# MangoSister/VolumetricTerrain

Measured on AMD Instinct MI355X. Metric: marching-cubes extraction throughput on a 1024^3 perlin3d grid (Mvoxels/s), higher is better.
Workload: dtype f32

## Files before the change

### volumetricterrain_amd/csrc/terrain.hip

```cpp
#include "terrain_edit.h"
#include "terrain_stamp.h"
#include <algorithm>
#include <array>
#include <cmath>
#include <cstring>

namespace vtmc {

__device__ __forceinline__ float clampf(float v, float lo, float hi)
{
    if (v < lo) v = lo;
    else if (v > hi) v = hi;
    return v;
}

__device__ __forceinline__ float lerp_unity(float a, float b, float t)
{
    t = t < 0.0f ? 0.0f : (t > 1.0f ? 1.0f : t);
    return a + (b - a) * t;
}

__device__ __forceinline__ float query_density(const TerrainModifierArgs &m, float px, float py, float pz)
{
    if (m.kind == 0) return m.p[0] - py;
    if (m.kind == 1) {
        const float dx = px - m.p[0], dy = py - m.p[1], dz = pz - m.p[2];
        return m.p[3] - __builtin_sqrtf(dx * dx + dy * dy + dz * dz);
    }
    const float sx = px - m.p[0], sy = py - m.p[1], sz = pz - m.p[2];
    const float proj = sx * m.p[3] + sy * m.p[4] + sz * m.p[5];
    const float sq = sx * sx + sy * sy + sz * sz;
    const float c = m.p[7] - __builtin_sqrtf(sq - proj * proj);
    float r = proj;
    const float b = m.p[6] - proj;
    if (b < r) r = b;
    if (c < r) r = c;
    return r;
}

__global__ __launch_bounds__(256) void terrain_fill_kernel(float *__restrict__ grid, long long n, uint64_t seed)
{
    const long long stride = (long long)gridDim.x * blockDim.x;
    for (long long i = (long long)blockIdx.x * blockDim.x + threadIdx.x; i < n; i += stride)
        grid[i] = terrain_uniform(seed, 0u, (uint64_t)i, 0u) - 2.0f;
}

__device__ __forceinline__ float column_term(const TerrainModifierArgs &m, float px, float pz)
{
    if (m.kind != 3) return 0.0f;
    const float wm1 = (float)(m.dims0 - 1), hm1 = (float)(m.dims1 - 1);
    float u = clampf(px, 0.0f, m.p[0]);
    u = u / m.p[0] * wm1;
    u = clampf(u, 0.0f, wm1);
    float v = clampf(pz, 0.0f, m.p[1]);
    v = v / m.p[1] * hm1;
    v = clampf(v, 0.0f, hm1);
    const int u0 = (int)floorf(u), u1 = (int)ceilf(u), v0 = (int)floorf(v), v1 = (int)ceilf(v);
    const float h00 = m.data[(size_t)u0 * m.dims1 + v0], h10 = m.data[(size_t)u1 * m.dims1 + v0];
    const float h01 = m.data[(size_t)u0 * m.dims1 + v1], h11 = m.data[(size_t)u1 * m.dims1 + v1];
    const float h0 = lerp_unity(h00, h01, v - (float)v0);
    const float h1 = lerp_unity(h10, h11, v - (float)v0);
    return lerp_unity(h0, h1, u - (float)u0);
}

template <bool kJournal>
__global__ __launch_bounds__(256) void terrain_modify_kernel(float *__restrict__ grid, float *__restrict__ image, TerrainShape sh, TerrainModifierArgs m)
{
    const BoxThread t;
    if (!t.inside(m)) return;
    const int x = m.lx + t.ix, z = m.lz + t.iz;
    const float px = (float)x * sh.scale + sh.origin[0];
    const float pz = (float)z * sh.scale + sh.origin[2];
    const float col = column_term(m, px, pz);
    const uint64_t row = box_index(m, t.ix, 0, t.iz);
    for (int iy = t.iy0, iy1 = t.iy1(m); iy < iy1; ++iy) {
        const int y = m.ly + iy;
        const float py = (float)y * sh.scale + sh.origin[1];
        const uint64_t sample = grid_index(sh, x, y, z);
        const float q = m.kind == 3 ? col - py : query_density(m, px, py, pz);
        const float md = clamp_drawn(q, sh.seed, m.event, sample, 0u);
        const float s = grid[sample];
        if (kJournal) image[row + (uint64_t)m.dx * (uint64_t)iy] = s;
        grid[sample] = csg_combine(sh, m.event, sample, m.add_or_erode, md, s);
    }
}

__global__ __launch_bounds__(256) void terrain_swap_kernel(uint32_t *__restrict__ grid, uint32_t *__restrict__ image, TerrainShape sh, TerrainBox b)
{
    const BoxThread t;
    if (!t.inside(b)) return;
    const uint64_t s0 = grid_index(sh, b.lx + t.ix, b.ly + t.iy0, b.lz + t.iz), j0 = box_index(b, t.ix, t.iy0, t.iz);
    const int iy1 = t.iy1(b);
    uint32_t g[kYRun], h[kYRun];
#pragma unroll
    for (int k = 0; k < kYRun; ++k)
        if (t.iy0 + k < iy1) {
            g[k] = grid[s0 + (uint64_t)sh.dim_x * k];
            h[k] = image[j0 + (uint64_t)b.dx * k];
        }
#pragma unroll
    for (int k = 0; k < kYRun; ++k)
        if (t.iy0 + k < iy1) {
            grid[s0 + (uint64_t)sh.dim_x * k] = h[k];
            image[j0 + (uint64_t)b.dx * k] = g[k];
        }
}

__global__ __launch_bounds__(256) void terrain_stage_kernel(const float *__restrict__ grid, float *__restrict__ stage, TerrainShape sh, TerrainBox h)
{
    const BoxThread t;
    if (!t.inside(h)) return;
    const int iy1 = t.iy1(h);
    const uint64_t s0 = grid_index(sh, h.lx + t.ix, h.ly + t.iy0, h.lz + t.iz), j0 = box_index(h, t.ix, t.iy0, t.iz);
    float v[kYRun];
#pragma unroll
    for (int k = 0; k < kYRun; ++k)
        if (t.iy0 + k < iy1) v[k] = grid[s0 + (uint64_t)sh.dim_x * k];
#pragma unroll
    for (int k = 0; k < kYRun; ++k)
        if (t.iy0 + k < iy1) stage[j0 + (uint64_t)h.dx * k] = v[k];
}

hipError_t launch_terrain_fill(float *grid, long long n, uint64_t seed, int n_cus, hipStream_t stream)
{
    long long wgs = (n + 255) / 256;
    if (wgs > (long long)n_cus * 16) wgs = (long long)n_cus * 16;
    if (wgs < 1) wgs = 1;
    return launch(terrain_fill_kernel, dim3((unsigned)wgs), dim3(256), 0, stream, grid, n, seed);
}

hipError_t launch_terrain_modify(float *grid, const TerrainShape &sh, const TerrainModifierArgs &m, hipStream_t stream)
{
    return box_empty(box_of(m)) ? hipSuccess : launch_box(terrain_modify_kernel<false>, box_of(m), stream, grid, (float *)nullptr, sh, m);
}

hipError_t launch_terrain_copy_box(const float *grid, float *dst, const TerrainShape &sh, const TerrainBox &b, hipStream_t stream)
{
    return launch_box(terrain_stage_kernel, b, stream, grid, dst, sh, b);
}

static int saturating_int(float f)
{
    return f <= -2147483648.0f ? INT32_MIN : (f >= 2147483648.0f ? INT32_MAX : (int)f);
}

static std::array<int, 3> block_counts(const TerrainShape &sh) { return {(sh.dim_x - 2) / 8, (sh.dim_y - 2) / 8, (sh.dim_z - 2) / 8}; }
template <class F>
static void for_each_block(const std::array<int, 3> &nb, F f)
{
    for (int bz = 0; bz < nb[2]; ++bz)
        for (int by = 0; by < nb[1]; ++by)
            for (int bx = 0; bx < nb[0]; ++bx) f(bx, by, bz);
}

TerrainModifierArgs sample_range(const TerrainShape &sh, const vtmc_modifier &md, int low[3], int up[3])
{
    TerrainModifierArgs a{};
    a.kind = md.kind;
    a.add_or_erode = md.add_or_erode ? 1 : 0;
    memcpy(a.p, md.p, sizeof a.p);
    const int top[3] = {sh.dim_x - 1, sh.dim_y - 1, sh.dim_z - 1};
    int ext[3];
    for (int k = 0; k < 3; ++k) {
        low[k] = std::max(saturating_int(std::floor((md.lower[k] - sh.origin[k]) / sh.scale)), 0);
        up[k] = std::min(saturating_int(std::ceil((md.upper[k] - sh.origin[k]) / sh.scale)), top[k]);
        const long long e = (long long)up[k] - (long long)low[k] + 1;
        ext[k] = e <= 0 || low[k] > top[k] ? 0 : (int)std::min<long long>(e, (long long)top[k] - low[k] + 1);
    }
    a.lx = low[0], a.ly = low[1], a.lz = low[2];
    a.dx = ext[0], a.dy = ext[1], a.dz = ext[2];
    return a;
}

TerrainBox bounds_box(const TerrainShape &sh, const float lower[3], const float upper[3])
{
    vtmc_modifier md{};
    for (int k = 0; k < 3; ++k) md.lower[k] = lower[k], md.upper[k] = upper[k];
    int low[3], up[3];
    return box_of(sample_range(sh, md, low, up));
}

static size_t mark_dirty_blocks(const int low[3], const int up[3], const std::array<int, 3> &nb, std::vector<uint8_t> &mark)
{
    int b0[3], b1[3];
    for (int k = 0; k < 3; ++k) {
        const long long lo = (long long)low[k] - 8, hi = up[k];
        const long long f = lo <= 0 ? 0 : (lo + 7) / 8;
        const long long l = std::min<long long>(hi < 0 ? -1 : hi / 8, nb[k] - 1);
        if (f > l) return 0;
        b0[k] = (int)f;
        b1[k] = (int)l;
    }
    size_t n_new = 0;
    for (int bz = b0[2]; bz <= b1[2]; ++bz)
        for (int by = b0[1]; by <= b1[1]; ++by) {
            uint8_t *row = &mark[(size_t)nb[0] * ((size_t)by + (size_t)nb[1] * bz)];
            for (int bx = b0[0]; bx <= b1[0]; ++bx) {
                n_new += !row[bx];
                row[bx] = 1;
            }
        }
    return n_new;
}

int stage_for_queue(vtmc_ctx *ctx, VtmcDevBuf &buf, const void *host, size_t bytes)
{
    VTMC_HIP(ctx, hipStreamSynchronize(ctx->stream));
    if (int rc = ensure(ctx, buf, bytes)) return rc;
    VTMC_HIP(ctx, hipMemcpy(buf.p, host, bytes, hipMemcpyHostToDevice));
    return VTMC_OK;
}

static int check_reference(vtmc_ctx *ctx, const vtmc_modifier &md, int32_t i)
{
    if (md.kind == VTMC_MOD_HEIGHTMAP && (!md.data || md.data_dims[0] < 1 || md.data_dims[1] < 1))
        return fail(ctx, VTMC_ERR_INVALID_ARG, "modifier %d: heightmap data / dims missing", i);
    return VTMC_OK;
}

static int apply_reference(vtmc_ctx *ctx, const vtmc_modifier &md, const TerrainModifierArgs &args, float *grid, float *image)
{
    TerrainModifierArgs a = args;
    if (md.kind == VTMC_MOD_HEIGHTMAP) {
        if (int rc = stage_for_queue(ctx, ctx->heightmap, md.data, sizeof(float) * (size_t)md.data_dims[0] * (size_t)md.data_dims[1])) return rc;
        a.data = (const float *)ctx->heightmap.p;
        a.dims0 = md.data_dims[0];
        a.dims1 = md.data_dims[1];
    }
    VTMC_HIP(ctx, launch_box(image ? terrain_modify_kernel<true> : terrain_modify_kernel<false>, box_of(a), ctx->stream, grid, image, ctx->tshape, a));
    return VTMC_OK;
}

static const ModifierKind kModifierKinds[] = {
    {VTMC_MOD_PLANE, check_reference, apply_reference},
    {VTMC_MOD_SPHERE, check_reference, apply_reference},
    {VTMC_MOD_CYLINDER, check_reference, apply_reference},
    {VTMC_MOD_HEIGHTMAP, check_reference, apply_reference},
    {VTMC_MOD_SMOOTH, check_brush, apply_smooth},
    {VTMC_MOD_FLATTEN, check_brush, apply_flatten},
    {VTMC_MOD_NOISE, check_noise, apply_noise},
    {VTMC_MOD_STAMP, check_stamp, apply_stamp},
    {VTMC_MOD_PATH, check_path, apply_path},
    {VTMC_MOD_DETACH, check_detach, apply_detach},
};

const ModifierKind *find_modifier_kind(int32_t kind)
{
    for (const ModifierKind &k : kModifierKinds)
        if (k.kind == kind) return &k;
    return nullptr;
}

static int check_modifier(vtmc_ctx *ctx, const vtmc_modifier &md, int32_t i)
{
    const ModifierKind *k = find_modifier_kind(md.kind);
    return k ? k->check(ctx, md, i) : fail(ctx, VTMC_ERR_INVALID_ARG, "modifier %d: unknown kind %d", i, md.kind);
}

static int extract_dirty(vtmc_ctx *ctx, const std::vector<uint8_t> &mark, size_t n_marked, int32_t *n_dirty_blocks, int32_t *tri_count)
{
    const TerrainShape &sh = ctx->tshape;
    const auto nb = block_counts(sh);
    ctx->dirty.clear();
    ctx->dirty_is_all = n_marked == mark.size();
    if (!ctx->dirty_is_all) {
        ctx->dirty.reserve(n_marked * 3);
        size_t id = 0;
        for_each_block(nb, [&](int bx, int by, int bz) {
            if (mark[id++]) ctx->dirty.insert(ctx->dirty.end(), {bx, by, bz});
        });
    }
    if (n_dirty_blocks) *n_dirty_blocks = (int32_t)n_marked;
    BlockSpace sp = dense_space((const float *)ctx->terrain.p, sh.dim_x - 2, sh.dim_y - 2, sh.dim_z - 2, 1, sh.dim_x, (int64_t)sh.dim_x * sh.dim_y, 1, 0);
    int n_volumes = 1;
    if (!ctx->dirty_is_all) {
        if (int rc = upload_block_list(ctx, ctx->dirty.data(), (int)n_marked, sp)) return rc;
        n_volumes = 0;
    }
    return extract_core(ctx, sp, n_volumes, ResultSource::TerrainDirty, tri_count);
}

void history_clear(vtmc_ctx *ctx)
{
    ctx->hist.clear();
    ctx->hist_done = 0;
}

int terrain_extract_all(vtmc_ctx *ctx, int32_t *n_dirty_blocks, int32_t *tri_count)
{
    const auto nb = block_counts(ctx->tshape);
    const std::vector<uint8_t> mark((size_t)nb[0] * nb[1] * nb[2], 1);
    return extract_dirty(ctx, mark, mark.size(), n_dirty_blocks, tri_count);
}

static size_t image_bytes(const TerrainBox &b) { return box_empty(b) ? 0 : ((size_t)4 * b.dx * b.dy * b.dz + 255) / 256 * 256; }

static VtmcHistoryStep plan_step(vtmc_ctx *ctx, const vtmc_modifier *mods, int32_t n_mods)
{
    VtmcHistoryStep st;
    st.boxes.resize((size_t)n_mods);
    for (int32_t i = 0; i < n_mods; ++i) {
        VtmcHistoryBox &hb = st.boxes[i];
        const TerrainModifierArgs a = sample_range(ctx->tshape, mods[i], hb.low, hb.up);
        hb.box = box_of(a);
        hb.off = st.bytes;
        st.bytes += image_bytes(hb.box);
    }
    const size_t cap = ctx->journal.bytes;
    if (st.bytes == 0 || st.bytes > cap) {
        if (st.bytes) history_clear(ctx);
        st.boxes.clear();
        return st;
    }
    ctx->hist.resize(ctx->hist_done);
    const size_t head = ctx->hist.empty() ? 0 : ctx->hist.back().off + ctx->hist.back().bytes;
    st.off = head + st.bytes <= cap ? head : 0;
    if (st.off == 0)
        while (!ctx->hist.empty() && ctx->hist.front().off >= head) ctx->hist.pop_front();
    while (!ctx->hist.empty() && ctx->hist.front().off < st.off + st.bytes && st.off < ctx->hist.front().off + ctx->hist.front().bytes)
        ctx->hist.pop_front();
    ctx->hist_done = ctx->hist.size();
    for (VtmcHistoryBox &hb : st.boxes) hb.off += st.off;
    return st;
}

static int32_t history_step(vtmc_ctx *ctx, bool undo, int32_t *n_dirty_blocks, int32_t *tri_count)
{
    if (!ctx) return VTMC_ERR_INVALID_ARG;
    if (!ctx->has_terrain) return fail(ctx, VTMC_ERR_NO_RESULT, "terrain_%s before terrain_init", undo ? "undo" : "redo");
    if (undo ? ctx->hist_done == 0 : ctx->hist_done == ctx->hist.size())
        return fail(ctx, VTMC_ERR_NO_RESULT, "nothing to %s", undo ? "undo" : "redo");
    VTMC_HIP(ctx, hipSetDevice(ctx->device));
    const size_t k = undo ? ctx->hist_done - 1 : ctx->hist_done;
    const VtmcHistoryStep &st = ctx->hist[k];
    const auto nb = block_counts(ctx->tshape);
    std::vector<uint8_t> mark((size_t)nb[0] * nb[1] * nb[2], 0);
    size_t n_marked = 0;
    const size_t n = st.boxes.size();
    for (size_t i = 0; i < n; ++i) {
        const VtmcHistoryBox &hb = st.boxes[undo ? n - 1 - i : i];
        if (!box_empty(hb.box))
            if (hipError_t e = launch_box(terrain_swap_kernel, hb.box, ctx->stream, (uint32_t *)ctx->terrain.p,
                                          (uint32_t *)((char *)ctx->journal.p + hb.off), ctx->tshape, hb.box)) {
                history_clear(ctx);
                VTMC_HIP(ctx, e);
            }
        if (n_marked < mark.size()) n_marked += mark_dirty_blocks(hb.low, hb.up, nb, mark);
    }
    ctx->hist_done = undo ? k : k + 1;
    return extract_dirty(ctx, mark, n_marked, n_dirty_blocks, tri_count);
}

}

using namespace vtmc;

extern "C" {

int32_t vtmc_terrain_init(vtmc_ctx *ctx, int32_t width, int32_t elevation, int32_t height, float voxel_scale,
                          const float terrain_origin[3], uint64_t seed)
{
    if (!ctx) return VTMC_ERR_INVALID_ARG;
    if (!terrain_origin) return fail(ctx, VTMC_ERR_INVALID_ARG, "terrain_origin is null");
    if (int rc = check_dims(ctx, width, elevation, height)) return rc;
    if (width + 1 > 1025 || elevation + 1 > 1025 || height + 1 > 1025)
        return fail(ctx, VTMC_ERR_DIMS, "too high resolution (exceeds 1025)");
    if (!(voxel_scale > 0.0f)) return fail(ctx, VTMC_ERR_INVALID_ARG, "voxel_scale must be positive");
    VTMC_HIP(ctx, hipSetDevice(ctx->device));
    ctx->has_terrain = false;
    ctx->result.valid = false;
    history_clear(ctx);
    material_drop(ctx);
    nav_drop(ctx);
    water_drop(ctx);
    TerrainShape sh{};
    sh.dim_x = width + 2;
    sh.dim_y = elevation + 2;
    sh.dim_z = height + 2;
    sh.scale = voxel_scale;
    memcpy(sh.origin, terrain_origin, sizeof sh.origin);
    sh.seed = seed;
    const long long n = (long long)sh.dim_x * sh.dim_y * sh.dim_z;
    if (int rc = ensure(ctx, ctx->terrain, sizeof(float) * (size_t)n)) return rc;
    VTMC_HIP(ctx, launch_terrain_fill((float *)ctx->terrain.p, n, seed, ctx->n_cus, ctx->stream));
    VTMC_HIP(ctx, hipStreamSynchronize(ctx->stream));
    ctx->tshape = sh;
    ctx->terrain_events = 0;
    ctx->dirty.clear();
    ctx->dirty_is_all = false;
    ctx->has_terrain = true;
    return VTMC_OK;
}

int32_t vtmc_terrain_update(vtmc_ctx *ctx, const vtmc_modifier *mods, int32_t n_mods, int32_t *n_dirty_blocks, int32_t *tri_count)
{
    if (!ctx) return VTMC_ERR_INVALID_ARG;
    if (!ctx->has_terrain) return fail(ctx, VTMC_ERR_NO_RESULT, "terrain_update before terrain_init");
    if (n_mods < 0 || (n_mods > 0 && !mods)) return fail(ctx, VTMC_ERR_INVALID_ARG, "mods is null or n_mods < 0");
    VTMC_HIP(ctx, hipSetDevice(ctx->device));
    const TerrainShape &sh = ctx->tshape;
    const auto nb = block_counts(sh);
    std::vector<uint8_t> mark((size_t)nb[0] * nb[1] * nb[2], 0);
    size_t n_marked = 0;
    VtmcHistoryStep step;
    if (ctx->journal.p) {
        for (int32_t i = 0; i < n_mods; ++i)
            if (int rc = check_modifier(ctx, mods[i], i)) return rc;
        step = plan_step(ctx, mods, n_mods);
    }
    const bool journaled = !step.boxes.empty();
    struct ClearOnFailure {
        vtmc_ctx *ctx;
        bool armed;
        ~ClearOnFailure()
        {
            if (armed) history_clear(ctx);
        }
    } guard{ctx, journaled};
    for (int32_t i = 0; i < n_mods; ++i) {
        const vtmc_modifier &md = mods[i];
        if (int rc = check_modifier(ctx, md, i)) return rc;
        int low[3], up[3];
        TerrainModifierArgs a = sample_range(sh, md, low, up);
        a.event = ++ctx->terrain_events;
        if (!box_empty(box_of(a))) {
            float *image = journaled ? (float *)((char *)ctx->journal.p + step.boxes[i].off) : nullptr;
            if (int rc = find_modifier_kind(md.kind)->apply(ctx, md, a, (float *)ctx->terrain.p, image)) return rc;
        }
        if (n_marked < mark.size()) n_marked += mark_dirty_blocks(low, up, nb, mark);
    }
    if (journaled) {
        ctx->hist.push_back(std::move(step));
        ctx->hist_done = ctx->hist.size();
    }
    const int rc = extract_dirty(ctx, mark, n_marked, n_dirty_blocks, tri_count);
    guard.armed = rc != VTMC_OK && journaled;
    return rc;
}

int32_t vtmc_terrain_set_history(vtmc_ctx *ctx, int64_t max_bytes)
{
    if (!ctx) return VTMC_ERR_INVALID_ARG;
    if (max_bytes < 0) return fail(ctx, VTMC_ERR_INVALID_ARG, "max_bytes < 0");
    VTMC_HIP(ctx, hipSetDevice(ctx->device));
    history_clear(ctx);
    if (ctx->journal.bytes != (size_t)max_bytes) {
        VTMC_HIP(ctx, hipStreamSynchronize(ctx->stream));
        ctx->journal.release();
        if (max_bytes > 0) {
            VTMC_HIP(ctx, hipMalloc(&ctx->journal.p, (size_t)max_bytes));
            ctx->journal.bytes = (size_t)max_bytes;
        }
    }
    return VTMC_OK;
}

int32_t vtmc_terrain_undo(vtmc_ctx *ctx, int32_t *n_dirty_blocks, int32_t *tri_count) { return history_step(ctx, true, n_dirty_blocks, tri_count); }

int32_t vtmc_terrain_redo(vtmc_ctx *ctx, int32_t *n_dirty_blocks, int32_t *tri_count) { return history_step(ctx, false, n_dirty_blocks, tri_count); }

int32_t vtmc_terrain_history(const vtmc_ctx *ctx, int32_t *n_undo, int32_t *n_redo, int64_t *bytes_used)
{
    if (!ctx) return VTMC_ERR_INVALID_ARG;
    if (n_undo) *n_undo = (int32_t)ctx->hist_done;
    if (n_redo) *n_redo = (int32_t)(ctx->hist.size() - ctx->hist_done);
    if (bytes_used) {
        int64_t b = 0;
        for (const VtmcHistoryStep &st : ctx->hist) b += (int64_t)st.bytes;
        *bytes_used = b;
    }
    return VTMC_OK;
}

int32_t vtmc_terrain_dirty_blocks(vtmc_ctx *ctx, int32_t *dst, int32_t capacity_blocks, int32_t *n_blocks)
{
    if (!ctx) return VTMC_ERR_INVALID_ARG;
    if (!ctx->has_terrain) return fail(ctx, VTMC_ERR_NO_RESULT, "terrain_dirty_blocks before terrain_init");
    const auto nb = block_counts(ctx->tshape);
    const size_t n = ctx->dirty_is_all ? (size_t)nb[0] * nb[1] * nb[2] : ctx->dirty.size() / 3;
    if (n_blocks) *n_blocks = (int32_t)n;
    if (!dst) return VTMC_OK;
    if ((size_t)std::max(capacity_blocks, 0) < n) return fail(ctx, VTMC_ERR_CAPACITY, "capacity %d < %zu dirty blocks", capacity_blocks, n);
    if (ctx->dirty_is_all)
        for_each_block(nb, [&](int bx, int by, int bz) {
            *dst++ = bx;
            *dst++ = by;
            *dst++ = bz;
        });
    else if (n)
        memcpy(dst, ctx->dirty.data(), n * 3 * sizeof(int32_t));
    return VTMC_OK;
}

int32_t vtmc_terrain_read_samples(vtmc_ctx *ctx, float *dst, int64_t stride_x, int64_t stride_y, int64_t stride_z)
{
    if (!ctx) return VTMC_ERR_INVALID_ARG;
    if (!ctx->has_terrain) return fail(ctx, VTMC_ERR_NO_RESULT, "terrain_read_samples before terrain_init");
    if (!dst) return fail(ctx, VTMC_ERR_INVALID_ARG, "dst is null");
    if (stride_x <= 0 || stride_y <= 0 || stride_z <= 0) return fail(ctx, VTMC_ERR_INVALID_ARG, "strides must be positive");
    VTMC_HIP(ctx, hipSetDevice(ctx->device));
    const TerrainShape &sh = ctx->tshape;
    const size_t n = (size_t)sh.dim_x * sh.dim_y * sh.dim_z;
    VTMC_HIP(ctx, hipStreamSynchronize(ctx->stream));
    if (stride_x == 1 && stride_y == sh.dim_x && stride_z == (int64_t)sh.dim_x * sh.dim_y) {
        VTMC_HIP(ctx, hipMemcpy(dst, ctx->terrain.p, n * sizeof(float), hipMemcpyDeviceToHost));
        return VTMC_OK;
    }
    std::vector<float> tmp(n);
    VTMC_HIP(ctx, hipMemcpy(tmp.data(), ctx->terrain.p, n * sizeof(float), hipMemcpyDeviceToHost));
    size_t i = 0;
    for (int z = 0; z < sh.dim_z; ++z)
        for (int y = 0; y < sh.dim_y; ++y)
            for (int x = 0; x < sh.dim_x; ++x) dst[x * stride_x + y * stride_y + z * stride_z] = tmp[i++];
    return VTMC_OK;
}

int32_t vtmc_terrain_device_grid(vtmc_ctx *ctx, const float **d_samples, int64_t strides[3], int32_t dims[3])
{
    if (!ctx) return VTMC_ERR_INVALID_ARG;
    if (!ctx->has_terrain) return fail(ctx, VTMC_ERR_NO_RESULT, "terrain_device_grid before terrain_init");
    const TerrainShape &sh = ctx->tshape;
    if (d_samples) *d_samples = (const float *)ctx->terrain.p;
    if (strides) {
        strides[0] = 1;
        strides[1] = sh.dim_x;
        strides[2] = (int64_t)sh.dim_x * sh.dim_y;
    }
    if (dims) {
        dims[0] = sh.dim_x;
        dims[1] = sh.dim_y;
        dims[2] = sh.dim_z;
    }
    return VTMC_OK;
}

}
```

### volumetricterrain_amd/csrc/terrain_box.h

```cpp
#ifndef VTMC_TERRAIN_BOX_H
#define VTMC_TERRAIN_BOX_H
#include "vtmc_ctx.h"
#include "terrain_hash.h"

namespace vtmc {

__device__ __forceinline__ float clamp_drawn(float v, uint64_t seed, uint32_t event, uint64_t sample, uint32_t k)
{
    if (v < -1.0f) {
        const float lo = terrain_uniform(seed, event, sample, k) - 2.0f;
        if (v < lo) v = lo;
    } else if (v > 1.0f) {
        const float hi = terrain_uniform(seed, event, sample, k + 1u) + 1.0f;
        if (v > hi) v = hi;
    }
    return v;
}

__device__ __forceinline__ float csg_combine(const TerrainShape &sh, uint32_t event, uint64_t sample, int add_or_erode, float md, float s)
{
    if (add_or_erode) return s > md ? s : md;
    const float minus_md = -md;
    return clamp_drawn(s < minus_md ? s : minus_md, sh.seed, event, sample, 2u);
}

constexpr int kYRun = 16;

struct BoxThread {
    int ix, iz, iy0;
    __device__ __forceinline__ BoxThread() : ix(blockIdx.x * 64 + threadIdx.x), iz(blockIdx.y * 4 + threadIdx.y), iy0(blockIdx.z * kYRun) {}
    template <class Box>
    __device__ __forceinline__ bool inside(const Box &b) const { return ix < b.dx && iz < b.dz; }
    template <class Box>
    __device__ __forceinline__ int iy1(const Box &b) const { return iy0 + kYRun < b.dy ? iy0 + kYRun : b.dy; }
};
__device__ __forceinline__ uint64_t grid_index(const TerrainShape &sh, int x, int y, int z)
{
    return (uint64_t)x + (uint64_t)sh.dim_x * ((uint64_t)y + (uint64_t)sh.dim_y * (uint64_t)z);
}
template <class Box>
__device__ __forceinline__ uint64_t box_index(const Box &b, int ix, int iy, int iz)
{
    return (uint64_t)ix + (uint64_t)b.dx * ((uint64_t)iy + (uint64_t)b.dy * (uint64_t)iz);
}

static bool box_empty(const TerrainBox &b) { return b.dx <= 0 || b.dy <= 0 || b.dz <= 0; }

static dim3 box_grid(const TerrainBox &b) { return dim3((unsigned)((b.dx + 63) / 64), (unsigned)((b.dz + 3) / 4), (unsigned)((b.dy + kYRun - 1) / kYRun)); }
static bool box_launchable(const TerrainBox &b) { return (b.dz + 3) / 4 <= 65535 && (b.dy + kYRun - 1) / kYRun <= 65535; }

template <class... Params, class... Args>
static hipError_t launch_box(void (*kernel)(Params...), const TerrainBox &b, hipStream_t stream, Args... args)
{
    return box_launchable(b) ? launch(kernel, box_grid(b), dim3(64, 4, 1), 0, stream, args...) : hipErrorInvalidValue;
}

}
#endif
```

### volumetricterrain_amd/csrc/terrain_edit.h

```cpp
#ifndef VTMC_TERRAIN_EDIT_H
#define VTMC_TERRAIN_EDIT_H
#include "terrain_box.h"

namespace vtmc {

struct ModifierKind {
    int32_t kind;
    int (*check)(vtmc_ctx *ctx, const vtmc_modifier &md, int32_t i);
    int (*apply)(vtmc_ctx *ctx, const vtmc_modifier &md, const TerrainModifierArgs &a, float *grid, float *image);
};
const ModifierKind *find_modifier_kind(int32_t kind);

int check_brush(vtmc_ctx *ctx, const vtmc_modifier &md, int32_t i);
int check_noise(vtmc_ctx *ctx, const vtmc_modifier &md, int32_t i);
int check_stamp(vtmc_ctx *ctx, const vtmc_modifier &md, int32_t i);
int check_path(vtmc_ctx *ctx, const vtmc_modifier &md, int32_t i);
int check_detach(vtmc_ctx *ctx, const vtmc_modifier &md, int32_t i);
int apply_smooth(vtmc_ctx *ctx, const vtmc_modifier &md, const TerrainModifierArgs &a, float *grid, float *image);
int apply_flatten(vtmc_ctx *ctx, const vtmc_modifier &md, const TerrainModifierArgs &a, float *grid, float *image);
int apply_noise(vtmc_ctx *ctx, const vtmc_modifier &md, const TerrainModifierArgs &a, float *grid, float *image);
int apply_stamp(vtmc_ctx *ctx, const vtmc_modifier &md, const TerrainModifierArgs &a, float *grid, float *image);
int apply_path(vtmc_ctx *ctx, const vtmc_modifier &md, const TerrainModifierArgs &a, float *grid, float *image);
int apply_detach(vtmc_ctx *ctx, const vtmc_modifier &md, const TerrainModifierArgs &a, float *grid, float *image);

static TerrainBox box_of(const TerrainModifierArgs &m) { return TerrainBox{m.lx, m.ly, m.lz, m.dx, m.dy, m.dz}; }
TerrainModifierArgs sample_range(const TerrainShape &sh, const vtmc_modifier &md, int low[3], int up[3]);
TerrainBox bounds_box(const TerrainShape &sh, const float lower[3], const float upper[3]);
int stage_for_queue(vtmc_ctx *ctx, VtmcDevBuf &buf, const void *host, size_t bytes);

}
#endif
```

### volumetricterrain_amd/csrc/vtmc_ctx.h

```cpp
#ifndef VTMC_CTX_H
#define VTMC_CTX_H
#include "../../include/vtmc.h"
#include "vtmc_internal.h"
struct vtmc_nav_span;
#include "../../include/vtmc_water.h"

#include <deque>
#include <map>
#include <string>
#include <utility>
#include <vector>

namespace vtmc {
struct TerrainBox {
    int lx, ly, lz;
    int dx, dy, dz;
};
template <typename T, hipError_t (*Free)(void *)>
struct OwnedBuf {
    T *p = nullptr;
    size_t bytes = 0;
    OwnedBuf() = default;
    OwnedBuf(OwnedBuf &&o) noexcept { swap(o); }
    OwnedBuf &operator=(OwnedBuf o) noexcept { return swap(o); }
    ~OwnedBuf() { release(); }
    OwnedBuf &swap(OwnedBuf &o) noexcept
    {
        std::swap(p, o.p);
        std::swap(bytes, o.bytes);
        return *this;
    }
    void release()
    {
        if (p) quiet(Free(p));
        p = nullptr;
        bytes = 0;
    }
};
template <int N>
struct StageClock {
    hipEvent_t ev[N] = {};
    bool armed = false;
    StageClock() = default;
    StageClock(const StageClock &) = delete;
    StageClock &operator=(const StageClock &) = delete;
    ~StageClock()
    {
        for (hipEvent_t e : ev)
            if (e) quiet(hipEventDestroy(e));
    }
    hipError_t begin()
    {
        armed = false;
        for (hipEvent_t &e : ev)
            if (!e)
                if (hipError_t rc = hipEventCreate(&e)) return rc;
        return hipSuccess;
    }
    hipError_t mark(int i, hipStream_t stream) { return hipEventRecord(ev[i], stream); }
    void arm() { armed = true; }
    hipEvent_t event(int i) const { return ev[i]; }
    int sync_last(vtmc_ctx *ctx) const;
    int elapsed(vtmc_ctx *ctx, int i, int j, float *ms) const;
};
}
typedef vtmc::OwnedBuf<void, hipFree> VtmcDevBuf;
template <typename T>
using VtmcPinnedBuf = vtmc::OwnedBuf<T, hipHostFree>;

struct VtmcHistoryBox {
    vtmc::TerrainBox box;
    int low[3], up[3];
    size_t off = 0;
};
struct VtmcHistoryStep {
    std::vector<VtmcHistoryBox> boxes;
    size_t off = 0, bytes = 0;
};

struct VtmcStamp {
    VtmcDevBuf samples;
    int nx = 0, ny = 0, nz = 0;
};

enum class ResultSource { Caller, TerrainDirty, TerrainLod };

struct VtmcResult {
    bool valid = false;
    uint64_t epoch = 0;
    ResultSource source = ResultSource::Caller;
    vtmc::BlockSpace space{};
    int blocks = 0;
    uint32_t active = 0;
    int volumes = 0;
    int64_t tris = 0, verts = 0;
    bool indexed = false;
    int64_t vertices() const { return indexed ? verts : 3 * tris; }
};

struct VertexAttr {
    VtmcDevBuf values;
    int64_t n = 0;
    uint64_t epoch = 0;
};

struct VtmcScatter {
    VtmcDevBuf instances, block_offsets, masks, tiles;
    int64_t n = 0;
    int blocks = 0;
    uint64_t epoch = 0;
};

struct VtmcNav {
    VtmcDevBuf spans, offsets, scan, scratch, ctl;
    VtmcDevBuf spans_next, offsets_next;
    bool valid = false;
    int32_t n = 0;
    int32_t lo[3] = {0, 0, 0}, d[3] = {0, 0, 0};
    int rounds = 0;
};

struct VtmcNavField {
    VtmcDevBuf cells, work, ctl;
    bool valid = false;
    int32_t n = 0, reached = 0, rounds = 0;
};

struct VtmcNavErode {
    VtmcDevBuf state, links, dist, remap, origin, ctl;
    bool dist_valid = false, origin_valid = false;
    int32_t dist_n = 0, origin_n = 0;
    int32_t rounds = 0;
};

struct VtmcNavCrowd {
    VtmcDevBuf agents, pending, occupancy, claims, links, ctl;
    bool valid = false;
    int32_t n_agents = 0, n_spans = 0;
    int32_t occupying = 0, arrived = 0, ticks = 0, moved_last = 0;
};

struct VtmcWater {
    VtmcDevBuf water, body, labels, records, seeds, source_body, ctl, probe;
    bool valid = false;
    int32_t lo[3] = {0, 0, 0}, d[3] = {0, 0, 0}, vd[3] = {0, 0, 0};
    int64_t wet = 0;
    std::vector<vtmc_water_body> bodies;
};

struct VtmcLodSkirt {
    VtmcDevBuf tris, node_offsets, masks, tiles, node_masks, sink;
    std::vector<uint8_t> face_masks;
    int64_t n = 0;
    int32_t nodes = 0, flagged = 0;
    uint64_t epoch = 0;
    bool staged = false;
};

struct VtmcPending {
    bool active = false;
    bool launched = false;
    vtmc::BlockSpace sp{};
    int n_volumes = 0;
    bool indexed = false;
    ResultSource source = ResultSource::Caller;
    hipStream_t stream = nullptr;
    size_t tcap = 0, vcap = 0;
    bool scan_event = false;
    bool counts_early = false;
};

struct vtmc_ctx {
    int device = 0;
    int n_cus = 256;
    hipStream_t stream = nullptr;
    bool stream_own_queue = false;
    hipStream_t queue_stream = nullptr;
    vtmc::DeviceTables tables{nullptr, nullptr};
    VtmcDevBuf d_vert, d_trinum;
    VtmcDevBuf counts, offsets, active, partials, totals, volcounts, cases, tris, input, list, perm, origins, yrows;
    VtmcDevBuf vcounts, voffsets, vtotals, verts, indices;
    int output_mode = VTMC_OUTPUT_SOUP;
    uint32_t *h_totals_dev = nullptr;
    VtmcPinnedBuf<uint32_t> h_totals;
    hipEvent_t ev[5] = {nullptr, nullptr, nullptr, nullptr, nullptr};
    VtmcDevBuf signs;
    struct {
        bool valid = false;
        const float *d_out = nullptr;
        int dx = 0, dy = 0, dz = 0, n_volumes = 0;
        long long sv = 0;
    } sign_of;
    VtmcPinnedBuf<float> h_stage;
    int h_stage_small_calls = 0;
    VtmcPinnedBuf<int32_t> h_origins;
    hipEvent_t ev_origins = nullptr;
    bool origins_upload_pending = false;
    float stage_ms[4] = {0, 0, 0, 0};
    bool place_pending = false;
    float place_ms[16] = {0, 0, 0, 0, 0, 0, 0, 0, 0, 0, 0, 0, 0, 0, 0, 0};
    int place_n = 0, place_kept = 0;
    vtmc::StageClock<2> fill_clock;
    VtmcPending pending;
    VtmcResult result;
    vtmc::Tuning tune;
    VtmcDevBuf terrain, heightmap;
    vtmc::TerrainShape tshape{};
    bool has_terrain = false;
    uint32_t terrain_events = 0;
    std::vector<int32_t> dirty;
    bool dirty_is_all = false;
    VtmcDevBuf journal;
    std::deque<VtmcHistoryStep> hist;
    size_t hist_done = 0;
    VtmcDevBuf brush;
    std::map<int32_t, VtmcStamp> stamps;
    int32_t next_stamp_id = 1;
    VtmcDevBuf path;
    VtmcDevBuf frag_labels, frag_ctl, frag_records;
    VtmcDevBuf material, mat_image, mat_strokes;
    int mat_c = 0;
    VertexAttr mat_weights;
    VertexAttr ao;
    VtmcDevBuf ao_stats;
    int32_t ao_direct_max = -1;
    VtmcScatter scatter;
    vtmc::StageClock<6> scatter_clock;
    VtmcNav nav;
    vtmc::StageClock<9> nav_clock;
    VtmcNavField navfield;
    vtmc::StageClock<4> navfield_clock;
    VtmcNavErode naverode;
    vtmc::StageClock<5> naverode_clock;
    VtmcDevBuf navsight_links;
    vtmc::StageClock<3> navsight_clock;
    VtmcNavCrowd navcrowd;
    vtmc::StageClock<2> navcrowd_clock;
    VtmcWater water;
    vtmc::StageClock<4> water_clock;
    std::vector<vtmc_lod_node> lod_nodes;
    VtmcDevBuf lod_nodes_dev, lod_tiles;
    vtmc::StageClock<2> lod_clock;
    VtmcLodSkirt lodskirt;
    vtmc::StageClock<6> lodskirt_clock;
    VtmcDevBuf rays;
    VtmcPinnedBuf<unsigned char> h_rays;
    uint64_t perm_seed = 0;
    bool perm_valid = false;
    VtmcDevBuf tio_bricks, tio_stage;
    VtmcPinnedBuf<unsigned char> h_tio;
    VtmcDevBuf chunk_image;
    bool comm_borrowed = false;
    void *comm = nullptr;
    int comm_rank = 0, comm_world = 1;
    VtmcDevBuf comm_send;
    hipStream_t comm_stream = nullptr;
    hipEvent_t ev_gather = nullptr;
    hipEvent_t ev_last_gather = nullptr;
    bool gather_recorded = false;
    hipEvent_t ev_comm_chain = nullptr;
    hipStream_t comm_chain_stream = nullptr;
    bool comm_chain_recorded = false;
    vtmc_ctx *comm_owner = nullptr;
    std::vector<vtmc_ctx *> comm_borrowers;
    std::string err;
};

namespace vtmc {
int fail(vtmc_ctx *ctx, int code, const char *fmt, ...) __attribute__((format(printf, 3, 4)));
int ensure(vtmc_ctx *ctx, VtmcDevBuf &b, size_t bytes);
inline void release(VtmcDevBuf &b) { b.release(); }
template <typename T>
hipError_t pin(VtmcPinnedBuf<T> &b, size_t bytes)
{
    b.release();
    const hipError_t e = hipHostMalloc((void **)&b.p, bytes, hipHostMallocDefault);
    if (e == hipSuccess) b.bytes = bytes;
    else b.p = nullptr;
    return e;
}
hipError_t take_stream(int device, bool own_queue, int n_cus, hipStream_t *out);
void comm_release(vtmc_ctx *ctx);
int check_dims(vtmc_ctx *ctx, int nx, int ny, int nz);
BlockSpace dense_space(const float *d_base, int nx, int ny, int nz, int64_t sx, int64_t sy, int64_t sz, int n_volumes, int64_t sv);
float *pinned_stage(vtmc_ctx *ctx, size_t bytes);
void material_drop(vtmc_ctx *ctx);
inline void nav_drop(vtmc_ctx *ctx) { ctx->nav.valid = false, ctx->navfield.valid = false, ctx->naverode.dist_valid = false, ctx->naverode.origin_valid = false, ctx->navcrowd.valid = false; }
inline void water_drop(vtmc_ctx *ctx) { ctx->water.valid = false; }
int upload_block_list(vtmc_ctx *ctx, const int32_t *xyz, int n, BlockSpace &sp);
int extract_core(vtmc_ctx *ctx, const BlockSpace &sp, int n_volumes, ResultSource source, int32_t *tri_count);
int attr_gate(vtmc_ctx *ctx, const char *who);
int attr_read(vtmc_ctx *ctx, const VertexAttr &a, const char *stale, size_t bytes_per_vertex, uint8_t *dst, int64_t capacity_vertices);
int attr_device_results(vtmc_ctx *ctx, const VertexAttr &a, const char *stale, const uint8_t **d_values, int64_t *n_vertices);
void history_clear(vtmc_ctx *ctx);
int terrain_extract_all(vtmc_ctx *ctx, int32_t *n_dirty_blocks, int32_t *tri_count);

struct ScanLayout;
hipError_t nav_launch_offsets(const ScanLayout &scan, int32_t *offsets, hipStream_t stream);
int nav_label_regions(vtmc_ctx *ctx, const char *who, vtmc_nav_span *spans, int32_t *parent, int32_t n, bool timed, int *rounds);
struct NavBox;
NavBox nav_held_box(const VtmcNav &nav);

struct TraceRows {
    const int32_t *starts;
    int32_t *paths, *lengths;
    size_t path_bytes, length_bytes, host_off;
};
int trace_rows_stage(vtmc_ctx *ctx, const int32_t *starts, int32_t n_starts, int32_t max_len, TraceRows *rows);
int trace_rows_fetch(vtmc_ctx *ctx, const TraceRows &rows, int32_t *paths, int32_t *lengths);

template <class... Params, class... Args>
hipError_t launch(void (*kernel)(Params...), dim3 grid, dim3 block, size_t lds_bytes, hipStream_t stream, Args... args)
{
    launch_begin();
    hipLaunchKernelGGL(kernel, grid, block, lds_bytes, stream, args...);
    return launch_end();
}
inline dim3 lanes256(int64_t n) { return dim3((unsigned)((n + 255) / 256)); }
}

#define VTMC_HIP(ctx, expr)                                                                                \
    do {                                                                                                   \
        hipError_t e_ = (expr);                                                                            \
        if (e_ != hipSuccess)                                                                              \
            return vtmc::fail(ctx, VTMC_ERR_DEVICE, "%s failed: %s (%s:%d)", #expr, hipGetErrorString(e_), \
                              __FILE__, __LINE__);                                                         \
    } while (0)

template <int N>
int vtmc::StageClock<N>::sync_last(vtmc_ctx *ctx) const
{
    VTMC_HIP(ctx, hipSetDevice(ctx->device));
    VTMC_HIP(ctx, hipEventSynchronize(ev[N - 1]));
    return VTMC_OK;
}
template <int N>
int vtmc::StageClock<N>::elapsed(vtmc_ctx *ctx, int i, int j, float *ms) const
{
    VTMC_HIP(ctx, hipEventElapsedTime(ms, ev[i], ev[j]));
    return VTMC_OK;
}

#endif
```

Baseline: 663,400.

## Batch non-overlapping plane/sphere/cylinder terrain modifiers into one kernel launch

Plane, sphere and cylinder modifiers are now queued instead of launched one at a time. They are grouped into dependency levels by box overlap, and up to sixteen modifiers per level go out in a single batched kernel that maps blocks to modifiers through prefix offsets. The modify kernel also loads its y-run of grid samples up front before computing. This targets launch overhead in terrain editing. The metric is marching-cubes extraction throughput, which this path likely does not touch, and the batching adds host-side reordering and per-block modifier lookup.

Measured after the change: 647,300. 2.4% lower.

```diff
diff --git a/volumetricterrain_amd/csrc/terrain.hip b/volumetricterrain_amd/csrc/terrain.hip
--- a/volumetricterrain_amd/csrc/terrain.hip
+++ b/volumetricterrain_amd/csrc/terrain.hip
@@ -64,25 +64,52 @@
 }
 
 template <bool kJournal>
-__global__ __launch_bounds__(256) void terrain_modify_kernel(float *__restrict__ grid, float *__restrict__ image, TerrainShape sh, TerrainModifierArgs m)
-{
-    const BoxThread t;
+__device__ __forceinline__ void modify_run(float *__restrict__ grid, float *__restrict__ image, const TerrainShape &sh, const TerrainModifierArgs &m, const BoxThread &t)
+{
     if (!t.inside(m)) return;
     const int x = m.lx + t.ix, z = m.lz + t.iz;
     const float px = (float)x * sh.scale + sh.origin[0];
     const float pz = (float)z * sh.scale + sh.origin[2];
     const float col = column_term(m, px, pz);
-    const uint64_t row = box_index(m, t.ix, 0, t.iz);
-    for (int iy = t.iy0, iy1 = t.iy1(m); iy < iy1; ++iy) {
-        const int y = m.ly + iy;
-        const float py = (float)y * sh.scale + sh.origin[1];
-        const uint64_t sample = grid_index(sh, x, y, z);
-        const float q = m.kind == 3 ? col - py : query_density(m, px, py, pz);
-        const float md = clamp_drawn(q, sh.seed, m.event, sample, 0u);
-        const float s = grid[sample];
-        if (kJournal) image[row + (uint64_t)m.dx * (uint64_t)iy] = s;
-        grid[sample] = csg_combine(sh, m.event, sample, m.add_or_erode, md, s);
-    }
+    const int n = t.iy1(m) - t.iy0;
+    const uint64_t s0 = grid_index(sh, x, m.ly + t.iy0, z);
+    const uint64_t j0 = box_index(m, t.ix, t.iy0, t.iz);
+    float s[kYRun];
+    load_run(s, grid + s0, (uint64_t)sh.dim_x, n);
+#pragma unroll
+    for (int k = 0; k < kYRun; ++k)
+        if (k < n) {
+            const int y = m.ly + t.iy0 + k;
+            const float py = (float)y * sh.scale + sh.origin[1];
+            const uint64_t sample = s0 + (uint64_t)sh.dim_x * k;
+            const float q = m.kind == 3 ? col - py : query_density(m, px, py, pz);
+            const float md = clamp_drawn(q, sh.seed, m.event, sample, 0u);
+            if (kJournal) image[j0 + (uint64_t)m.dx * k] = s[k];
+            grid[sample] = csg_combine(sh, m.event, sample, m.add_or_erode, md, s[k]);
+        }
+}
+
+template <bool kJournal>
+__global__ __launch_bounds__(256) void terrain_modify_kernel(float *__restrict__ grid, float *__restrict__ image, TerrainShape sh, TerrainModifierArgs m)
+{
+    modify_run<kJournal>(grid, image, sh, m, BoxThread());
+}
+
+constexpr int kModifyBatch = 16;
+struct ModifyBatch {
+    TerrainModifierArgs m[kModifyBatch];
+    float *image[kModifyBatch];
+    unsigned first[kModifyBatch];
+};
+template <bool kJournal>
+__global__ __launch_bounds__(256) void terrain_modify_batch_kernel(float *__restrict__ grid, TerrainShape sh, ModifyBatch b)
+{
+    int j = 0;
+#pragma unroll
+    for (int k = 1; k < kModifyBatch; ++k) j += blockIdx.x >= b.first[k];
+    const TerrainModifierArgs &m = b.m[j];
+    const unsigned w = blockIdx.x - b.first[j], gx = (unsigned)(m.dx + 63) / 64, gz = (unsigned)(m.dz + 3) / 4;
+    modify_run<kJournal>(grid, kJournal ? b.image[j] : nullptr, sh, m, BoxThread(w % gx, w / gx % gz, w / gx / gz));
 }
 
 __global__ __launch_bounds__(256) void terrain_swap_kernel(uint32_t *__restrict__ grid, uint32_t *__restrict__ image, TerrainShape sh, TerrainBox b)
@@ -218,24 +245,77 @@
     return VTMC_OK;
 }
 
-static int apply_reference(vtmc_ctx *ctx, const vtmc_modifier &md, const TerrainModifierArgs &args, float *grid, float *image)
+static hipError_t launch_modify(vtmc_ctx *ctx, const TerrainModifierArgs &a, float *image)
+{
+    return launch_box(image ? terrain_modify_kernel<true> : terrain_modify_kernel<false>, box_of(a), ctx->stream, (float *)ctx->terrain.p, image, ctx->tshape, a);
+}
+
+static int apply_heightmap(vtmc_ctx *ctx, const vtmc_modifier &md, const TerrainModifierArgs &args, float *, float *image)
 {
     TerrainModifierArgs a = args;
-    if (md.kind == VTMC_MOD_HEIGHTMAP) {
-        if (int rc = stage_for_queue(ctx, ctx->heightmap, md.data, sizeof(float) * (size_t)md.data_dims[0] * (size_t)md.data_dims[1])) return rc;
-        a.data = (const float *)ctx->heightmap.p;
-        a.dims0 = md.data_dims[0];
-        a.dims1 = md.data_dims[1];
-    }
-    VTMC_HIP(ctx, launch_box(image ? terrain_modify_kernel<true> : terrain_modify_kernel<false>, box_of(a), ctx->stream, grid, image, ctx->tshape, a));
+    if (int rc = stage_for_queue(ctx, ctx->heightmap, md.data, sizeof(float) * (size_t)md.data_dims[0] * (size_t)md.data_dims[1])) return rc;
+    a.data = (const float *)ctx->heightmap.p;
+    a.dims0 = md.data_dims[0];
+    a.dims1 = md.data_dims[1];
+    VTMC_HIP(ctx, launch_modify(ctx, a, image));
+    return VTMC_OK;
+}
+
+static int apply_reference(vtmc_ctx *ctx, const vtmc_modifier &, const TerrainModifierArgs &a, float *, float *image)
+{
+    ctx->stretch.push_back({a, image});
+    return VTMC_OK;
+}
+
+static bool boxes_overlap(const TerrainModifierArgs &a, const TerrainModifierArgs &b)
+{
+    return a.lx < b.lx + b.dx && b.lx < a.lx + a.dx && a.ly < b.ly + b.dy && b.ly < a.ly + a.dy && a.lz < b.lz + b.dz && b.lz < a.lz + a.dz;
+}
+
+static int flush_stretch(vtmc_ctx *ctx)
+{
+    std::vector<VtmcQueuedModifier> q;
+    q.swap(ctx->stretch);
+    const size_t n = q.size();
+    std::vector<int> level(n, 0);
+    std::vector<size_t> order(n);
+    for (size_t i = 0; i < n; ++i) {
+        order[i] = i;
+        for (size_t j = 0; j < i; ++j)
+            if (level[j] >= level[i] && boxes_overlap(q[j].a, q[i].a)) level[i] = level[j] + 1;
+    }
+    std::stable_sort(order.begin(), order.end(), [&](size_t x, size_t y) { return level[x] < level[y]; });
+    for (size_t at = 0; at < n;) {
+        ModifyBatch b{};
+        uint64_t wgs = 0;
+        size_t k = 0;
+        for (; k < kModifyBatch && at + k < n && level[order[at + k]] == level[order[at]]; ++k) {
+            const VtmcQueuedModifier &qm = q[order[at + k]];
+            const dim3 g = box_grid(box_of(qm.a));
+            const uint64_t own = (uint64_t)g.x * g.y * g.z;
+            if (k > 0 && wgs + own > 0x7fffffffu) break;
+            b.m[k] = qm.a;
+            b.image[k] = qm.image;
+            b.first[k] = (unsigned)wgs;
+            wgs += own;
+        }
+        if (k == 1) {
+            VTMC_HIP(ctx, launch_modify(ctx, b.m[0], b.image[0]));
+        } else {
+            for (size_t r = k; r < kModifyBatch; ++r) b.first[r] = UINT32_MAX;
+            VTMC_HIP(ctx, launch(b.image[0] ? terrain_modify_batch_kernel<true> : terrain_modify_batch_kernel<false>, dim3((unsigned)wgs), dim3(64, 4, 1), 0,
+                                 ctx->stream, (float *)ctx->terrain.p, ctx->tshape, b));
+        }
+        at += k;
+    }
     return VTMC_OK;
 }
 
 static const ModifierKind kModifierKinds[] = {
-    {VTMC_MOD_PLANE, check_reference, apply_reference},
-    {VTMC_MOD_SPHERE, check_reference, apply_reference},
-    {VTMC_MOD_CYLINDER, check_reference, apply_reference},
-    {VTMC_MOD_HEIGHTMAP, check_reference, apply_reference},
+    {VTMC_MOD_PLANE, check_reference, apply_reference, true},
+    {VTMC_MOD_SPHERE, check_reference, apply_reference, true},
+    {VTMC_MOD_CYLINDER, check_reference, apply_reference, true},
+    {VTMC_MOD_HEIGHTMAP, check_reference, apply_heightmap},
     {VTMC_MOD_SMOOTH, check_brush, apply_smooth},
     {VTMC_MOD_FLATTEN, check_brush, apply_flatten},
     {VTMC_MOD_NOISE, check_noise, apply_noise},
@@ -417,18 +497,27 @@
             if (armed) history_clear(ctx);
         }
     } guard{ctx, journaled};
-    for (int32_t i = 0; i < n_mods; ++i) {
-        const vtmc_modifier &md = mods[i];
-        if (int rc = check_modifier(ctx, md, i)) return rc;
-        int low[3], up[3];
-        TerrainModifierArgs a = sample_range(sh, md, low, up);
-        a.event = ++ctx->terrain_events;
-        if (!box_empty(box_of(a))) {
-            float *image = journaled ? (float *)((char *)ctx->journal.p + step.boxes[i].off) : nullptr;
-            if (int rc = find_modifier_kind(md.kind)->apply(ctx, md, a, (float *)ctx->terrain.p, image)) return rc;
-        }
-        if (n_marked < mark.size()) n_marked += mark_dirty_blocks(low, up, nb, mark);
-    }
+    const auto walk = [&]() -> int {
+        for (int32_t i = 0; i < n_mods; ++i) {
+            const vtmc_modifier &md = mods[i];
+            if (int rc = check_modifier(ctx, md, i)) return rc;
+            const ModifierKind *kind = find_modifier_kind(md.kind);
+            if (!kind->enqueues)
+                if (int rc = flush_stretch(ctx)) return rc;
+            int low[3], up[3];
+            TerrainModifierArgs a = sample_range(sh, md, low, up);
+            a.event = ++ctx->terrain_events;
+            if (!box_empty(box_of(a))) {
+                float *image = journaled ? (float *)((char *)ctx->journal.p + step.boxes[i].off) : nullptr;
+                if (int rc = kind->apply(ctx, md, a, (float *)ctx->terrain.p, image)) return rc;
+            }
+            if (n_marked < mark.size()) n_marked += mark_dirty_blocks(low, up, nb, mark);
+        }
+        return VTMC_OK;
+    };
+    const int walked = walk(), flushed = flush_stretch(ctx);
+    if (walked) return walked;
+    if (flushed) return flushed;
     if (journaled) {
         ctx->hist.push_back(std::move(step));
         ctx->hist_done = ctx->hist.size();
diff --git a/volumetricterrain_amd/csrc/terrain_box.h b/volumetricterrain_amd/csrc/terrain_box.h
--- a/volumetricterrain_amd/csrc/terrain_box.h
+++ b/volumetricterrain_amd/csrc/terrain_box.h
@@ -28,7 +28,8 @@
 
 struct BoxThread {
     int ix, iz, iy0;
-    __device__ __forceinline__ BoxThread() : ix(blockIdx.x * 64 + threadIdx.x), iz(blockIdx.y * 4 + threadIdx.y), iy0(blockIdx.z * kYRun) {}
+    __device__ __forceinline__ BoxThread() : BoxThread(blockIdx.x, blockIdx.y, blockIdx.z) {}
+    __device__ __forceinline__ BoxThread(unsigned bx, unsigned bz, unsigned by) : ix(bx * 64 + threadIdx.x), iz(bz * 4 + threadIdx.y), iy0(by * kYRun) {}
     template <class Box>
     __device__ __forceinline__ bool inside(const Box &b) const { return ix < b.dx && iz < b.dz; }
     template <class Box>
@@ -44,6 +45,14 @@
     return (uint64_t)ix + (uint64_t)b.dx * ((uint64_t)iy + (uint64_t)b.dy * (uint64_t)iz);
 }
 
+template <class T>
+__device__ __forceinline__ void load_run(T (&v)[kYRun], const T *p, uint64_t stride, int n)
+{
+#pragma unroll
+    for (int k = 0; k < kYRun; ++k)
+        if (k < n) v[k] = p[stride * k];
+}
+
 static bool box_empty(const TerrainBox &b) { return b.dx <= 0 || b.dy <= 0 || b.dz <= 0; }
 
 static dim3 box_grid(const TerrainBox &b) { return dim3((unsigned)((b.dx + 63) / 64), (unsigned)((b.dz + 3) / 4), (unsigned)((b.dy + kYRun - 1) / kYRun)); }
diff --git a/volumetricterrain_amd/csrc/terrain_edit.h b/volumetricterrain_amd/csrc/terrain_edit.h
--- a/volumetricterrain_amd/csrc/terrain_edit.h
+++ b/volumetricterrain_amd/csrc/terrain_edit.h
@@ -8,6 +8,7 @@
     int32_t kind;
     int (*check)(vtmc_ctx *ctx, const vtmc_modifier &md, int32_t i);
     int (*apply)(vtmc_ctx *ctx, const vtmc_modifier &md, const TerrainModifierArgs &a, float *grid, float *image);
+    bool enqueues = false;
 };
 const ModifierKind *find_modifier_kind(int32_t kind);
 
diff --git a/volumetricterrain_amd/csrc/vtmc_ctx.h b/volumetricterrain_amd/csrc/vtmc_ctx.h
--- a/volumetricterrain_amd/csrc/vtmc_ctx.h
+++ b/volumetricterrain_amd/csrc/vtmc_ctx.h
@@ -76,6 +76,11 @@
 struct VtmcHistoryStep {
     std::vector<VtmcHistoryBox> boxes;
     size_t off = 0, bytes = 0;
+};
+
+struct VtmcQueuedModifier {
+    vtmc::TerrainModifierArgs a;
+    float *image;
 };
 
 struct VtmcStamp {
@@ -213,6 +218,7 @@
     VtmcDevBuf journal;
     std::deque<VtmcHistoryStep> hist;
     size_t hist_done = 0;
+    std::vector<VtmcQueuedModifier> stretch;
     VtmcDevBuf brush;
     std::map<int32_t, VtmcStamp> stamps;
     int32_t next_stamp_id = 1;
```
